# mattsaccount364/FractalShark

Hardware: AMD Instinct MI355X
Metric: Mpix/s (iteration buffer), View #5 3840x2160 HDRx32 LAv2 (higher is better)
Workload: dtype f32+i32exp; 1 GPU; view5_3840x2160_hdrx32_lav2_full; parity=cpu, kernel_variant=tuned, frames=warm: frames of one view back to back

## Files before the change

### fractalshark_amd/csrc/kernels_lav2_hdr32.hip

```cpp
#include <hip/hip_runtime.h>
#include <stdint.h>

#include <type_traits>

#include "../../include/fs_layout.h"
#include "hdr_math.hpp"
#include "at_math.hpp"
#include "kernels.h"
#include <cstdlib>
#include "kernel_common.hpp"
#include "lav2_common.hpp"
#include "scaled_runs.hpp"

using namespace fs;

__global__ void k_test_block_threshold(const int *__restrict__ bw, const int *__restrict__ eshm, const int *__restrict__ sdc,
                                       int *__restrict__ t_out, uint32_t n)
{
    const uint32_t i = blockIdx.x;
    if (i >= n)
        return;
    const int b = __builtin_amdgcn_readfirstlane(bw[i]), e = __builtin_amdgcn_readfirstlane(eshm[i]),
              d = __builtin_amdgcn_readfirstlane(sdc[i]);
    int t;
// ... 19 lines not shown
    if (A.tile_order) {
        const uint32_t w = (blockIdx.y * gridDim.x + blockIdx.x) * (blockDim.x >> 6) + wave_in_block;
        const uint32_t tile = (uint32_t)__builtin_amdgcn_readfirstlane((int)A.tile_order[w]);
        tile_y = tile != 0xFFFFFFFFu ? tile / A.tiles_x : 0u;
        tile_x = tile != 0xFFFFFFFFu ? tile - tile_y * A.tiles_x : 0xFFFFFFFu;
    } else {
        tile_x = blockIdx.x * (blockDim.x >> 6) + wave_in_block;
        tile_y = blockIdx.y;
    }
    uint32_t X, L;
    uint32_t lds_lane16 = 0;
    {
        uint32_t lane;
        asm volatile("v_mbcnt_lo_u32_b32 %0, -1, 0\n\tv_mbcnt_hi_u32_b32 %0, -1, %0" : "=v"(lane));
        X = tile_x * 8u + (lane & 7u);
        L = tile_y * 8u + (lane >> 3);
        if constexpr (kLds)
            asm volatile("v_lshlrev_b32_e32 %0, 4, %1" : "=v"(lds_lane16) : "v"(lane));
    }
    uint32_t lane_cost = 0;
#ifdef FS_TRACE_WAVES
    const uint64_t trace_t0 = wall_clock64();
#endif
    uint64_t c_at = 0, c_la = 0, c_pt = 0, c_px = 0;
    uint64_t c_careful = 0, c_scaled = 0, c_runs = 0;
    uint32_t c_why[4] = {0, 0, 0, 0};
    uint32_t c_nz[4] = {0, 0, 0, 0};
    bool was_skip = false;
    uint32_t c_wentry = 0, c_wstart = 0, c_wshort = 0;
    uint32_t c_blk_violation = 0;
    uint32_t c_pass = 0, c_generic = 0;
    uint32_t c_blk_free = 0, c_blk_tested = 0;
    uint32_t c_lane_steps = 0, c_lane_runs = 0;
#ifdef FS_PROFILE_CYCLES
    uint64_t cyc_loop = 0, cyc_run = 0, cyc_body = 0, cyc_t0 = 0, cyc_t1 = 0, cyc_t2 = 0;
    uint64_t cyc_asm = 0, cyc_tested = 0, cyc_hot = 0, cyc_t3 = 0, cyc_t4 = 0, cyc_t5 = 0, wall_loop = 0, wall_t0 = 0;
#define FS_CYC(stmt) do { if (kStats) { stmt; } } while (0)
#else
#define FS_CYC(stmt) do { } while (0)
#endif
    const uint32_t Y = global_row(A.frame, L);
    const bool live = X < A.frame.width && L < A.frame.local_rows && Y < A.frame.height;
    if (live) {
        c_px = 1;
        const uint32_t n_iterations = A.n_iterations;
        hreal32 deltaReal, deltaImaginary;
        pixel_delta<float>(A.coords, X, Y, deltaReal, deltaImaginary);
        const hcplx32 DeltaSub0 = hc_from_hr(deltaReal, deltaImaginary);
        hcplx32 DeltaSubN = hc_from_native<float>(0.0f, 0.0f);
        uint32_t iterations = 0;
        uint32_t la_cost = 0;

        if (Mode != FS_MODE_PO) {
            if (A.la_valid && A.use_at && hr_cmp_pos(hc_cheb(DeltaSub0), ldr(A.at.ThresholdC)) <= 0) {
                const uint32_t ATMaxIt = n_iterations / A.at.StepLength;
                hcplx32 c = hc_add(hc_mul(DeltaSub0, ldc(A.at.CCoeff)), ldc(A.at.RefC));
                hc_reduce(c);
                hcplx32 z;
                uint32_t i;
                at_perform<float>(c, ldr(A.at.SqrEscapeRadius), ATMaxIt, z, i);
                hcplx32 dz = hc_mul(z, ldc(A.at.InvZCoeff));
                hc_reduce(dz);
                DeltaSubN = dz;
                iterations = i * A.at.StepLength;
                la_cost = i;
                if (kStats)
// ... 86 lines not shown
                pd[0] = dc.re, pd[1] = dc.im, pd[2] = __int_as_float(dc.e);
            }
            int sdc_bits;
            {
                const float mdc = fs_max_abs(dc.re, dc.im);
                const int de = dc.e < -400 ? -400 : (dc.e > 400 ? 400 : dc.e);
                const int lane_bits = mdc > 0.0f ? __float_as_int(__builtin_fmaxf(__builtin_amdgcn_ldexpf(mdc, de), 0x1p-126f))
                                                 : (mdc == 0.0f ? 0 : 0x7f800000);
                sdc_bits = wave_upper_bound_i32(lane_bits);
            }
#define FS_LOAD_DC()                                                                                                \
    f2 dcm;                                                                                                         \
    int dce;                                                                                                        \
    {                                                                                                               \
        uint32_t lane_d;                                                                                            \
        asm volatile("v_mbcnt_lo_u32_b32 %0, -1, 0\n\tv_mbcnt_hi_u32_b32 %0, -1, %0" : "=v"(lane_d));             \
        const uint32_t dc_addr_ = (uint32_t)(uintptr_t)(__attribute__((address_space(3))) float4 *)s_dcp +          \
                                  ((wave_in_block * 64u + lane_d) << 4);                                            \
        typedef float f3l_ __attribute__((ext_vector_type(3)));                                                     \
        f3l_ dc3_;                                                                                                  \
        asm volatile("ds_read_b96 %0, %1\n\ts_waitcnt lgkmcnt(0)" : "=v"(dc3_) : "v"(dc_addr_) : "memory");       \
        dcm = (f2){dc3_.x, dc3_.y};                                                                                 \
        dce = __float_as_int(dc3_.z);                                                                               \
    }
            auto pow2_or_zero = [](int g) -> float {
                return g > -kExpDiffIgnored ? __int_as_float((int)(((uint32_t)g << 23) + 0x3F800000u)) : 0.0f;
            };
            const float4 *__restrict__ zq = A.zq;
            const float4 *__restrict__ zs = A.zs;
            FS_CYC(cyc_t0 = __builtin_readcyclecounter());
            FS_CYC(wall_t0 = wall_clock64());
            uint32_t sc_skip = 0, sc_penalty = 0;
            bool fl_per_trip = false;
            while (running) {
                bool sc_stopped = false;
                if (kScaled && sc_skip != 0u) {
                    bool hot_progress = false, hot_cold = false;
                    FS_CYC(cyc_t5 = __builtin_readcyclecounter());
                    {
                        FS_LOAD_DC()
                        const int E = dze + kScaleShift;
                        const float sE = __builtin_amdgcn_ldexpf(1.0f, E);
                        const f2 sE2 = {sE, sE};
                        const int dsh = dce - E;
                        const f2 dcs = {__builtin_amdgcn_ldexpf(dcm.x, dsh), __builtin_amdgcn_ldexpf(dcm.y, dsh)};
                        const float4 e0 = zs[ref];
                        const float mx0 = fs_max_abs(dzm.x, dzm.y);
                        const float mn0 = fs_min_abs(dzm.x, dzm.y);
                        const bool start_ok = scaled_startable(e0) && mn0 >= FS_FL_FLOOR * __builtin_amdgcn_ldexpf(1.0f, kScaleShift) &&
                                              mx0 >= 1.0f && mx0 < 2.0f && dsh <= 30 - kScaleShift;
                        if (__builtin_amdgcn_ballot_w64(!start_ok) == 0ull) {
                            f2 w = dzm * __builtin_amdgcn_ldexpf(1.0f, -kScaleShift);
                            bool live = true;
#pragma unroll 1
                            for (uint32_t budget = kHotRunSteps; budget != 0u; budget--) {
                                f2 q_, zt;
                                float nz, nq, mxq, mnq, entz;
                                int hb;
                                {
                                    const uint32_t off_ = (live ? ref + 1u : 1u) << 4;
                                    asm volatile("global_load_dwordx2 v[58:59], %[off], %[zs] offset:-16\n\t"
                                                 "global_load_dwordx3 v[60:62], %[off], %[zs]\n\t"
                                                 "s_waitcnt vmcnt(0)\n\t"
                                                 "v_pk_fma_f32 v[56:57], %[w], %[se], v[58:59]\n\t"
                                                 "v_mul_f32_e32 v50, 0.5, v60\n\t"
                                                 "v_pk_mul_f32 v[58:59], %[w], v[56:57] op_sel_hi:[0,1]\n\t"
// ... 119 lines not shown
#define FS_TRIP_FAILED(T, NW_, EB, WSTART)                                                                         \
    {                                                                                                               \
        const float mn_s = fs_min_abs(NW_.x, NW_.y);                         \
        const uint64_t bad_s =                                                                                      \
            __builtin_amdgcn_ballot_w64(__float_as_int(mx_##T) + Esh > __float_as_int(EB)) |                        \
            __builtin_amdgcn_ballot_w64(!(mn_s >= FS_FL_FLOOR));                                                    \
        if (bad_s == 0ull) {                                                                                        \
            wO = NW_;                                                                                               \
            c += 1;                                                                                                 \
        } else {                                                                                                    \
            wO = WSTART;                                                                                            \
        }                                                                                                           \
        failed = true;                                                                                              \
    }
#define FS_TRIP_FAILED_NB(T, NW_, EB, WSTART)                                                                      \
    {                                                                                                               \
        const float mx_s = fs_max_abs(NW_.x, NW_.y);                         \
        const float mn_s = fs_min_abs(NW_.x, NW_.y);                         \
        const uint64_t bad_s =                                                                                      \
            __builtin_amdgcn_ballot_w64(__float_as_int(mx_s) + Esh > __float_as_int(EB)) |                        \
            __builtin_amdgcn_ballot_w64(!(mn_s >= FS_FL_FLOOR));                                                  \
        if (bad_s == 0ull) {                                                                                        \
            wO = NW_;                                                                                               \
            c += 1;                                                                                                 \
        } else {                                                                                                    \
            wO = WSTART;                                                                                            \
        }                                                                                                           \
        failed = true;                                                                                              \
    }
                        f2 w0 = dzm * __builtin_amdgcn_ldexpf(1.0f, -kScaleShift), z0 = {e0.x, e0.y}, w2, z2, wO;
                        uint32_t c = 0;
                        bool failed;
                        FS_CYC(cyc_t2 = __builtin_readcyclecounter());
                        bool fl_redo = false;
                        const uint32_t ref_u = (uint32_t)__builtin_amdgcn_readfirstlane((int)ref);
                        if (__builtin_amdgcn_ballot_w64(ref != ref_u) == 0ull) {
                            if constexpr (kLds) {
                                float4 *wbuf = s_zs_lds + (threadIdx.x >> 6) * 128u;
                                const uint32_t lds_base = (uint32_t)__builtin_amdgcn_readfirstlane(
                                    (int)(uint32_t)(uintptr_t)(__attribute__((address_space(3))) float4 *)wbuf);
                                const uint32_t nchunks = (run_len + 63u) >> 6;
#define FS_GLDS_CHUNK(CH)                                                                                           \
    {                                                                                                               \
        const float4 *src_ = zs + (ref_u + 1u + (CH) * 64u);   \
        const uint32_t dst_ = lds_base + (((CH) & 1u) << 10);                                                       \
        uint32_t keep_;                                                                                             \
        uint64_t exec_;                                                                                             \
        asm volatile("s_or_saveexec_b64 %0, -1\n\t"                                                               \
                     "s_mov_b32 %1, m0\n\t"                                                                       \
                     "s_mov_b32 m0, %3\n\t"                                                                       \
                     "s_nop 0\n\t"                                                                                \
                     "global_load_lds_dwordx4 %2, %4\n\t"                                                         \
                     "s_mov_b32 m0, %1\n\t"                                                                       \
                     "s_mov_b64 exec, %0"                                                                           \
                     : "=&s"(exec_), "=&s"(keep_)                                                                   \
                     : "v"(lds_lane16), "s"(dst_), "s"(src_)                                                        \
                     : "memory", "scc");                                                                            \
    }
                                FS_GLDS_CHUNK(0u)
                                uint32_t chunk = 0;
                                bool run_over = false;
                                while (!run_over) {
                                    if (chunk + 1u < nchunks) {
                                        FS_GLDS_CHUNK(chunk + 1u)
                                        asm volatile("s_waitcnt vmcnt(1)" ::: "memory");
                                    } else {
                                        asm volatile("s_waitcnt vmcnt(0)" ::: "memory");
// ... 31 lines not shown
                                            FS_TRIP_FAILED(e, t5, ue.z, w0)
                                            run_over = true;
                                            break;
                                        }
                                        c += 2;
                                        f2 t7, u7;
                                        uint64_t v4 = 0;
                                        FS_SCALED_STEP(w2, z2, t7, u7, g, v4, false, (void)0, ug.x, ug.y, ug.z);
                                        FS_SCALED_STEP(t7, u7, w0, z0, h, v4, true, (void)0, uh.x, uh.y, uh.z);
                                        if (v4 != 0ull) {
                                            FS_TRIP_FAILED(g, t7, ug.z, w2)
                                            run_over = true;
                                            break;
                                        }
                                        c += 2;
                                    }
                                    if (run_over)
                                        break;
                                    chunk++;
                                    if (c >= run_len) {
                                        wO = w0, failed = false;
                                        run_over = true;
                                    }
                                }
                                asm volatile("s_waitcnt vmcnt(0)" ::: "memory");
#undef FS_GLDS_CHUNK
                            } else {
                            typedef float f4 __attribute__((ext_vector_type(4)));
                            const float4 *zpu = zs + ref_u + 1;
#if defined(FS_VERIFY_BLOCK_BOUND) || defined(FS_VERIFY_FLOOR)
                            const int imdc = __float_as_int(fs_max_abs(dcs.x, dcs.y));
#endif
                            const int Esh_cap = wave_upper_bound_i32(Esh);
                            float mxS = mx0 * __builtin_amdgcn_ldexpf(1.0f, -kScaleShift);
                            int pwi = __builtin_amdgcn_readfirstlane(__float_as_int(e0.w));
                            f2 zS = {__int_as_float(__builtin_amdgcn_readfirstlane(__float_as_int(e0.x))),
                                     __int_as_float(__builtin_amdgcn_readfirstlane(__float_as_int(e0.y)))};
                            f2 wv = w0;
                            uint32_t cs = 0;
                            const uint32_t rl = (uint32_t)__builtin_amdgcn_readfirstlane((int)run_len);
                            const uint32_t lim8 = (rl << 4) - 0x80u;
                            const float4 *const zpb = zpu;
                            for (;;) {
#ifdef FS_VERIFY_BLOCK_BOUND
                                const long long bt_d = (long long)pwi - (long long)Esh_cap;
                                const int bt_thr = sdc_bits > pwi ? -1 : (bt_d > 0x46800000ll ? 0x46800000 : (int)bt_d);
                                const bool bt_pass = __builtin_amdgcn_ballot_w64(__float_as_int(mxS) > bt_thr) == 0ull;
                                if (kStats && bt_pass)
                                    c_blk_free++;
#else
                                {
                                    f2 r1, r2, r3 = wv, ts_, ta_;
                                    uint64_t xacc_ = 0;
                                    float tn_, tl_;
                                    uint64_t msk_;
                                    int st, ebo, pf_, pg_, ph_, bt_t_;
                                    const uint32_t c_in = cs;
                                    uint32_t off = cs << 4;
                                    FS_CYC(cyc_t3 = __builtin_readcyclecounter());
#ifndef FS_VERIFY_FLOOR
                                    if (!fl_per_trip) {
                                        {
                                            FS_FAST_LOOP_FDU(FS_PF_NONE);
                                        }
                                        ebo = 0;
                                    } else
#endif
                                    {
#if !(defined(FS_VERIFY_BLOCK_BOUND) || defined(FS_VERIFY_FLOOR))
                                        const int imdc = __float_as_int(fs_max_abs(dcs.x, dcs.y));
#endif
                                        FS_FAST_LOOP_FL(FS_PF_NONE);
                                    }
#ifdef FS_VERIFY_FLOOR
                                    if (kStats && xacc_ != 0ull)
                                        c_blk_violation++;
#endif
                                    FS_CYC(cyc_asm += __builtin_readcyclecounter() - cyc_t3);
                                    st = __builtin_amdgcn_readfirstlane(st);
                                    zS = (f2){__int_as_float(__builtin_amdgcn_readfirstlane(__float_as_int(zS.x))),
                                              __int_as_float(__builtin_amdgcn_readfirstlane(__float_as_int(zS.y)))};
                                    if (st == 3) {
                                        fl_redo = true;
                                        break;
                                    }
                                    cs = (uint32_t)__builtin_amdgcn_readfirstlane((int)off) >> 4;
                                    pwi = __builtin_amdgcn_readfirstlane(pwi);
                                    if (kStats)
                                        c_blk_free += (cs - c_in) >> 2;
                                    if (st != 0) {
                                        const float ebf = __int_as_float(__builtin_amdgcn_readfirstlane(ebo));
                                        c = cs;
                                        if (st == 1) {
                                            FS_TRIP_FAILED_NB(a, r1, ebf, wv)
                                        } else {
                                            FS_TRIP_FAILED_NB(a, r3, ebf, r2)
                                        }
                                        break;
                                    }
                                }
#endif
                                if (cs + 4u > rl) {
                                    c = cs, wO = wv, failed = false;
                                    break;
                                }
                                if (__builtin_amdgcn_ballot_w64(!(mxS < FS_FL_HIGH)) != 0ull) {
                                    c = cs, wO = wv, failed = false;
                                    break;
                                }
                                if (kStats)
                                    c_blk_tested++;
                                FS_CYC(cyc_t4 = __builtin_readcyclecounter());
                                typedef float f16 __attribute__((ext_vector_type(16)));
                                f16 U;
                                asm volatile("s_load_dwordx16 %0, %1, 0x0" : "=s"(U) : "s"(zpb + cs));
                                f2 tp_, tq_;
                                FS_STEP_ARITH(wv, zS, tp_, a)
                                asm volatile("s_waitcnt lgkmcnt(0)" : "+s"(U), "+v"(tp_));
                                const f4 ua = U.s0123, ub = U.s4567, uc = U.s89ab, ud = U.scdef;
// ... 70 lines not shown
                                FS_SCALED_STEP(w2, z2, t3, u3, c_, v2, false,
                                               asm volatile("s_waitcnt vmcnt(1)" : "+v"(ent_c_), "+v"(mx_c_)), ent_c_.x,
                                               ent_c_.y, ent_c_.z);
                                FS_SCALED_STEP(t3, u3, w0, z0, d, v2, true,
                                               asm volatile("s_waitcnt vmcnt(0)" : "+v"(ent_d), "+v"(mx_d)), ent_d.x,
                                               ent_d.y, ent_d.z);
                                if (v2 != 0ull) {
                                    FS_TRIP_FAILED(c_, t3, ent_c_.z, w2)
                                    break;
                                }
                                c += 2;
                                zp += 4;
                                if (c >= run_len) {
                                    wO = w0, failed = false;
                                    break;
                                }
                            }
                            asm volatile("s_waitcnt vmcnt(0) ; scaled run, loop exit" ::"v"(ent_a), "v"(ent_b), "v"(ent_c_), "v"(ent_d));
                            if (kStats) {
                                c_lane_steps += c;
                                c_lane_runs++;
                            }
                        }
#undef FS_TRIP_FAILED
#undef FS_TRIP_FAILED_NB
                        FS_CYC(cyc_body += __builtin_readcyclecounter() - cyc_t2);
                        if (fl_redo) {
                            uint32_t lane_p;
                            asm volatile("v_mbcnt_lo_u32_b32 %0, -1, 0\n\tv_mbcnt_hi_u32_b32 %0, -1, %0" : "=v"(lane_p));
                            const volatile __attribute__((address_space(3))) float *pz =
                                (const volatile __attribute__((address_space(3))) float *)s_dzp + (wave_in_block * 64u + lane_p) * 2u;
                            dzm = (f2){pz[0], pz[1]};
                            dze = E - kScaleShift;
                            fl_per_trip = true;
                            continue;
                        }
                        fl_per_trip = false;
                        {
                            const float mxw = fs_max_abs(wO.x, wO.y);
                            const int k = (int)((uint32_t)__float_as_int(mxw) >> 23) - 127;
                            dzm = (f2){__builtin_amdgcn_ldexpf(wO.x, -k), __builtin_amdgcn_ldexpf(wO.y, -k)};
                            dze = E + k;
                            ref += c;
                            iterations += c;
                            if (kStats && c != 0u) {
                                c_pt += c;
                                c_scaled += c;
                                c_runs++;
                                c_wstart++;
                                if (c < 8u)
                                    c_wshort++;
                            }
                        }
                        if (failed) {
                            sc_stopped = true;
                            if (c == 0u) {
                                sc_penalty = sc_penalty < kScaledBackoffCap ? sc_penalty + 1u : kScaledBackoffCap;
                                sc_skip = sc_penalty;
                            } else if (c >= 8u) {
                                sc_penalty = 0u;
                            }
                            break;
                        }
                    }
                    FS_CYC(cyc_run += __builtin_readcyclecounter() - cyc_t1);
                }
#define FS_QUIET_STEP(DZM, DZE, ZCM, SC, W, NDZM, NDZE, NZCM, NSC, NW, K, VIOL)                                     \
// ... 236 lines not shown
#ifdef FS_PROFILE_CYCLES
    if (kStats) {
        if ((threadIdx.x & 63) == 0) {
            atomicAdd((unsigned long long *)&A.stats[0], (unsigned long long)cyc_loop);
            atomicAdd((unsigned long long *)&A.stats[1], (unsigned long long)cyc_run);
            atomicAdd((unsigned long long *)&A.stats[3], (unsigned long long)cyc_body);
            atomicAdd((unsigned long long *)&A.stats[24], (unsigned long long)cyc_asm);
            atomicAdd((unsigned long long *)&A.stats[25], (unsigned long long)cyc_tested);
            atomicAdd((unsigned long long *)&A.stats[26], (unsigned long long)cyc_hot);
            atomicAdd((unsigned long long *)&A.stats[27], (unsigned long long)wall_loop);
        }
        c_at = c_la = c_px = 0;
    }
#endif
    if (kStats) {
        add_stats(A.stats, c_at, c_la, c_pt, c_px);
        for (int off = 32; off > 0; off >>= 1) {
            c_careful += __shfl_down(c_careful, off);
            c_scaled += __shfl_down(c_scaled, off);
            c_runs += __shfl_down(c_runs, off);
            const uint32_t bf = __shfl_down(c_blk_free, off), bt = __shfl_down(c_blk_tested, off);
            c_blk_free = bf > c_blk_free ? bf : c_blk_free;
            c_blk_tested = bt > c_blk_tested ? bt : c_blk_tested;
            const uint32_t cp = __shfl_down(c_pass, off), cg = __shfl_down(c_generic, off);
            c_pass = cp > c_pass ? cp : c_pass;
            c_generic = cg > c_generic ? cg : c_generic;
            const uint32_t we = __shfl_down(c_wentry, off), ws = __shfl_down(c_wstart, off), wh = __shfl_down(c_wshort, off);
            c_wentry = we > c_wentry ? we : c_wentry;
            c_wstart = ws > c_wstart ? ws : c_wstart;
            c_wshort = wh > c_wshort ? wh : c_wshort;
            const uint32_t ls = __shfl_down(c_lane_steps, off), lr = __shfl_down(c_lane_runs, off);
            c_lane_steps = ls > c_lane_steps ? ls : c_lane_steps;
            c_lane_runs = lr > c_lane_runs ? lr : c_lane_runs;
            const uint32_t bv = __shfl_down(c_blk_violation, off);
            c_blk_violation = bv > c_blk_violation ? bv : c_blk_violation;
            for (int i = 0; i < 4; i++) {
                const uint32_t y = __shfl_down(c_why[i], off);
                c_why[i] = y > c_why[i] ? y : c_why[i];
                const uint32_t y2 = __shfl_down(c_nz[i], off);
                c_nz[i] = y2 > c_nz[i] ? y2 : c_nz[i];
            }
        }
        if ((threadIdx.x & 63) == 0) {
            atomicAdd((unsigned long long *)&A.stats[5], (unsigned long long)c_careful);
            atomicAdd((unsigned long long *)&A.stats[6], (unsigned long long)c_scaled);
            atomicAdd((unsigned long long *)&A.stats[7], (unsigned long long)c_runs);
            atomicAdd((unsigned long long *)&A.stats[8], (unsigned long long)c_blk_free);
            atomicAdd((unsigned long long *)&A.stats[9], (unsigned long long)c_blk_tested);
            atomicAdd((unsigned long long *)&A.stats[10], (unsigned long long)c_pass);
            atomicAdd((unsigned long long *)&A.stats[11], (unsigned long long)c_generic);
            atomicAdd((unsigned long long *)&A.stats[12], (unsigned long long)c_wentry);
            atomicAdd((unsigned long long *)&A.stats[13], (unsigned long long)c_wstart);
            atomicAdd((unsigned long long *)&A.stats[14], (unsigned long long)c_wshort);
            atomicAdd((unsigned long long *)&A.stats[15], (unsigned long long)c_blk_violation);
            for (int i = 0; i < 4; i++) {
                atomicAdd((unsigned long long *)&A.stats[16 + i], (unsigned long long)c_why[i]);
                atomicAdd((unsigned long long *)&A.stats[20 + i], (unsigned long long)c_nz[i]);
            }
            atomicAdd((unsigned long long *)&A.stats[28], (unsigned long long)c_lane_steps);
            atomicAdd((unsigned long long *)&A.stats[29], (unsigned long long)c_lane_runs);
        }
    }
}
#undef FS_CYC

static dim3 tile_grid(const FsFrame &f) { return dim3((f.width + 31) / 32, (f.local_rows + 7) / 8, 1); }

uint32_t fsk_lav2_hdr32_slots(const FsFrame &f)
{
    return ((f.width + 31u) / 32u) * 4u * ((f.local_rows + 7u) / 8u);
}

void fsk_lav2_hdr32(const FsLav2Args32 &A, int mode, bool stats, int variant, hipStream_t s)
{
    const bool lds_orbit = (variant & FS_VARIANT_FLAG_LDS_ORBIT) != 0;
    variant &= FS_VARIANT_BASE_MASK;
    const dim3 b(256), g = tile_grid(A.frame);
#define FS_LAUNCH_FAST(M, SC, LDS)                                                                                  \
    if (stats) {                                                                                                    \
        if (gs)                                                                                                     \
            hipLaunchKernelGGL((k_lav2_hdr32_fast<M, true, SC, LDS, true>), g, b, 0, s, A);                         \
        else                                                                                                        \
            hipLaunchKernelGGL((k_lav2_hdr32_fast<M, true, SC, LDS, false>), g, b, 0, s, A);                        \
    } else {                                                                                                        \
        if (gs)                                                                                                     \
            hipLaunchKernelGGL((k_lav2_hdr32_fast<M, false, SC, LDS, true>), g, b, 0, s, A);                        \
        else                                                                                                        \
            hipLaunchKernelGGL((k_lav2_hdr32_fast<M, false, SC, LDS, false>), g, b, 0, s, A);                       \
    }
#define FS_LAUNCH(M)                                                                                                \
    do {                                                                                                            \
        if (variant == FS_VARIANT_LITERAL) {                                                                        \
            fsk_lav2_lit32(A, M, stats, g, b, s);                       \
// ... 22 lines not shown
```

### fractalshark_amd/csrc/scaled_runs.hpp

```cpp
#pragma once

#include <hip/hip_runtime.h>
#include <stdint.h>

#include "hdr_math.hpp"
#include "kernels.h"

namespace {

static __device__ __forceinline__ float fs_max_abs(float a, float b)
{
    float r;
    asm("v_max_f32_e64 %0, |%1|, |%2|" : "=v"(r) : "v"(a), "v"(b));
    return r;
}
static __device__ __forceinline__ float fs_min_abs(float a, float b)
{
    float r;
    asm("v_min_f32_e64 %0, |%1|, |%2|" : "=v"(r) : "v"(a), "v"(b));
    return r;
}

}

// ... 133 lines not shown
        "s_branch .Lfl_end_%=\n"                                                                                    \
        ".Lfl_f2_%=:\n\t"                                                                                           \
        "s_mov_b32 %[st], 2\n\t"                                                                                    \
        "s_mov_b32 %[eb], s46\n\t"                                                                                  \
        "s_add_u32 %[off], %[off], 0x20\n\t"                                                                        \
        "s_branch .Lfl_end_%=\n"                                                                                    \
        ".Lfl_f3_%=:\n\t"                                                                                           \
        "s_mov_b32 %[st], 1\n\t"                                                                                    \
        "s_mov_b32 %[eb], s54\n\t"                                                                                  \
        "s_add_u32 %[off], %[off], 0x40\n"                                                                          \
        ".Lfl_end_%=:\n\t"                                                                                          \
        "s_waitcnt lgkmcnt(0)"         \
        : "+{v[48:49]}"(wv), "={v[50:51]}"(r1), "={v[52:53]}"(r2), "+{v[54:55]}"(r3), "={v[56:57]}"(ts_),           \
          "={v[58:59]}"(ta_), "+{v60}"(mxS), "={v61}"(tn_), "={v62}"(tl_), [m] "=&s"(msk_), [st] "=&s"(st),         \
          [eb] "=&s"(ebo), "+{s67}"(pwi), "+{s[64:65]}"(zS), [off] "+s"(off), [pf] "=&s"(pf_), [pg] "=&s"(pg_),     \
          [ph] "=&s"(ph_), [xa] "+s"(xacc_)                                                                         \
        : [se] "v"(sE2), [dc] "v"(dcs), [esh] "v"(Esh), [imdc] "v"(imdc), [lim8] "s"(lim8), "{s[68:69]}"(zpb),      \
          [flr] "s"(kFloorBits), [flr56] "s"((127 - 56) << 23)                                                      \
        : "s36", "s37", "s38", "s39", "s40", "s41", "s42", "s43", "s44", "s45", "s46", "s47", "s48", "s49", "s50",  \
          "s51", "s52", "s53", "s54", "s55", "s56", "s57", "s58", "s59", "s60", "s61", "s62", "s63", "s66", "vcc",  \
          "scc")

#define FS_FL_ACC(A, B) "v_min3_f32 v61, |" A "|, |" B "|, v61\n\t"
#define FS_BT_DC_MAX "v_max_i32_e32 v62, v60, %[imdc]\n\t"
#define FS_BT_DC_ADD "v_add_u32_e32 v62, v62, %[esh]\n\t"

#define FS_BT_T(BW)                                                                                                 \
    "s_sub_i32 %[t], " BW ", %[eshm]\n\t"                                                                           \
    "s_cselect_b32 %[t], 0x46800000, %[t]\n\t"                                                                      \
    "s_min_i32 %[t], %[t], 0x46800000\n\t"                                                                          \
    "s_cmp_gt_i32 %[sdc], " BW "\n\t"                                                                               \
    "s_cselect_b32 %[t], -1, %[t]\n\t"
#define FS_BT_V "v_cmp_lt_i32_e32 vcc, %[t], v60\n\t"
#define FS_FAST_LOOP_FDU(PF)                                                                                        \
    asm volatile(                                                                                                   \
        "v_mov_b32_e32 v61, 0x7f800000\n\t" FS_BT_T("s67") FS_BT_V                                                  \
        ".Lfu_loop_%=:\n\t"          \
        "s_cmp_gt_u32 %[off], %[lim8]\n\t"                                                                          \
        "s_cbranch_scc1 .Lfu_out_%=\n\t"                                                                            \
        "s_cbranch_vccnz .Lfu_out_%=\n\t"                                                         \
        FS_PK_F(FS_R0, "s[64:65]")                                                                                  \
        "s_load_dwordx16 s[36:51], s[68:69], %[off]\n\t"                                                            \
        "s_load_dwordx16 s[52:67], s[68:69], %[off] offset:0x40\n\t"                                                \
        FS_PK_MA(FS_R0) FS_PK_MB(FS_R0) FS_PK_P FS_PK_A(FS_R1)                                                      \
        "s_waitcnt lgkmcnt(0)\n\t" PF FS_BT_T("s51")                                                                \
        FS_PK_F(FS_R1, "s[36:37]") FS_FL_ACC("v50", "v51") FS_PK_MA(FS_R1) FS_PK_MB(FS_R1) FS_PK_P FS_PK_A(FS_R2)   \
        FS_PK_F(FS_R2, "s[40:41]") FS_FL_ACC("v52", "v53") FS_PK_MA(FS_R2) FS_PK_MB(FS_R2) FS_PK_P FS_PK_A(FS_R3)   \
        FS_PK_F(FS_R3, "s[44:45]") FS_FL_ACC("v54", "v55") FS_PK_MA(FS_R3) FS_PK_MB(FS_R3) FS_PK_P FS_PK_A(FS_R0)   \
         \
        FS_PK_F(FS_R0, "s[48:49]") FS_FL_ACC("v48", "v49") FS_PK_MA(FS_R0) FS_T_X("v48", "v49") FS_PK_MB(FS_R0)     \
        FS_PK_P FS_PK_A(FS_R1)                                                                                      \
        FS_PK_F(FS_R1, "s[52:53]") FS_BT_V FS_PK_MA(FS_R1) FS_PK_MB(FS_R1) FS_PK_P                                  \
        "s_cbranch_vccnz .Lfu_blk_%=\n\t" FS_PK_A(FS_R2)                                                            \
        FS_PK_F(FS_R2, "s[56:57]") FS_FL_ACC("v50", "v51") FS_PK_MA(FS_R2) FS_FL_ACC("v52", "v53") FS_PK_MB(FS_R2)  \
        FS_PK_P FS_PK_A(FS_R3)                                                                                      \
        FS_PK_F(FS_R3, "s[60:61]") FS_FL_ACC("v54", "v55") FS_PK_MA(FS_R3) FS_PK_MB(FS_R3) FS_PK_P FS_PK_A(FS_R0)   \
        "s_add_u32 %[off], %[off], 0x80\n\t" FS_BT_T("s67")                                                         \
        FS_T_X("v48", "v49") FS_FL_ACC("v48", "v49") FS_BT_V "s_branch .Lfu_loop_%=\n"                              \
        ".Lfu_blk_%=:\n\t"          \
        "s_mov_b64 s[64:65], s[48:49]\n\t"                                                                          \
        "s_mov_b32 s67, s51\n\t"                                                                                    \
        "s_add_u32 %[off], %[off], 0x40\n"                                                                          \
        ".Lfu_out_%=:\n\t"                                     \
        "s_mov_b32 %[st], 0\n\t" FS_FL_C                                                                            \
        "s_cbranch_vccz .Lfu_end_%=\n\t"                                                                            \
        "s_mov_b32 %[st], 3\n"                                                                                      \
        ".Lfu_end_%=:\n\t"                                                                                          \
        "s_waitcnt lgkmcnt(0)"                                                                                      \
        : "+{v[48:49]}"(wv), "={v[50:51]}"(r1), "={v[52:53]}"(r2), "={v[54:55]}"(r3), "={v[56:57]}"(ts_),           \
          "={v[58:59]}"(ta_), "+{v60}"(mxS), "={v61}"(tn_), [t] "=&s"(bt_t_), [st] "=&s"(st),                       \
          "+{s67}"(pwi), "+{s[64:65]}"(zS), [off] "+s"(off), [pf] "=&s"(pf_), [pg] "=&s"(pg_), [ph] "=&s"(ph_)      \
        : [se] "v"(sE2), [dc] "v"(dcs), [eshm] "s"(Esh_cap), [sdc] "s"(sdc_bits), [lim8] "s"(lim8),                 \
          "{s[68:69]}"(zpb), [flr] "s"(kFloorBits)                                                                  \
        : "s36", "s37", "s38", "s39", "s40", "s41", "s42", "s43", "s44", "s45", "s46", "s47", "s48", "s49", "s50",  \
          "s51", "s52", "s53", "s54", "s55", "s56", "s57", "s58", "s59", "s60", "s61", "s62", "s63", "s66", "vcc",  \
          "scc")

#define FS_FD16_TAIL(EC, ED)                                                                                        \
    FS_PK_F(FS_R2, EC) FS_FL_ACC("v50", "v51") FS_PK_MA(FS_R2) FS_FL_ACC("v52", "v53") FS_PK_MB(FS_R2)              \
    FS_PK_P FS_PK_A(FS_R3)                                                                                          \
    FS_PK_F(FS_R3, ED) FS_FL_ACC("v54", "v55") FS_PK_MA(FS_R3) FS_PK_MB(FS_R3) FS_PK_P FS_PK_A(FS_R0)

#define FS_FD16D_PAIR(EA, EB_, BW, WAIT, LOADS)                                                                     \
    FS_PK_F(FS_R0, EA) FS_FL_ACC("v48", "v49") FS_PK_MA(FS_R0)                                                      \
    "v_max3_f32 v62, |v48|, |v49|, %[imdc]\n\t"                                                                     \
    FS_PK_MB(FS_R0) FS_PK_P                                                                                         \
    "v_subrev_u32_e32 v45, 0x46800000, v62\n\t"                                                                     \
    FS_PK_A(FS_R1)                                                                                                  \
    "v_add_u32_e32 v62, v62, %[esh]\n\t" WAIT                                                                       \
    FS_PK_F(FS_R1, EB_)                                                                                             \
    "v_sub_i32 v62, v62, " BW " clamp\n\t"                                                                          \
    FS_PK_MA(FS_R1)                                                                                                 \
    "v_max3_i32 v63, v63, v62, v45\n\t"                                                                             \
    FS_PK_MB(FS_R1) FS_PK_P LOADS FS_PK_A(FS_R2)
#define FS_FAST_LOOP_FD16P                                                                                          \
    asm volatile(                                                                                                   \
        "v_mov_b32_e32 v61, 0x7f800000\n\t"  \
        "v_bfrev_b32_e32 v63, 1\n\t"                                                                                \
        "s_lshr_b32 %[oc], %[off], 1\n\t"                                                                           \
        "s_load_dwordx16 s[36:51], s[68:69], %[oc]\n\t"                                                             \
        "s_load_dwordx2 s[72:73], s[70:71], %[off]\n"                                                               \
        ".Lfp_loop_%=:\n\t"  \
        "v_sub_u32_e32 v45, %[flr], v61\n\t"                                                                        \
        FS_BT_DC_MAX "s_cmp_gt_u32 %[off], %[lim16]\n\t"                                                            \
        "v_max_i32_e32 v45, v45, v63\n\t"                                                                           \
        FS_BT_DC_ADD                                                                                                \
        "v_cmp_lt_i32_e32 vcc, 0, v45\n\t"                                                                          \
        "s_cbranch_vccnz .Lfp_redo_%=\n\t"                                                 \
        "s_cbranch_scc1 .Lfp_out_%=\n\t"                   \
// ... 140 lines not shown
```

Baseline: 191.2 Mpix/s.

## Add no-dc fast loop variant that drops delta-c add when provably negligible

```diff
diff --git a/fractalshark_amd/csrc/kernels_lav2_hdr32.hip b/fractalshark_amd/csrc/kernels_lav2_hdr32.hip
--- a/fractalshark_amd/csrc/kernels_lav2_hdr32.hip
+++ b/fractalshark_amd/csrc/kernels_lav2_hdr32.hip
@@ -75,6 +75,7 @@
     uint32_t c_pass = 0, c_generic = 0;
     uint32_t c_blk_free = 0, c_blk_tested = 0;
     uint32_t c_lane_steps = 0, c_lane_runs = 0;
+    uint32_t c_nd_steps = 0, c_nd_fail = 0, c_nd_replayed = 0, c_nd_mismatch = 0;
 #ifdef FS_PROFILE_CYCLES
     uint64_t cyc_loop = 0, cyc_run = 0, cyc_body = 0, cyc_t0 = 0, cyc_t1 = 0, cyc_t2 = 0;
     uint64_t cyc_asm = 0, cyc_tested = 0, cyc_hot = 0, cyc_t3 = 0, cyc_t4 = 0, cyc_t5 = 0, wall_loop = 0, wall_t0 = 0;
@@ -227,6 +228,7 @@
             FS_CYC(wall_t0 = wall_clock64());
             uint32_t sc_skip = 0, sc_penalty = 0;
             bool fl_per_trip = false;
+            uint32_t nd_skip = 0;
             while (running) {
                 bool sc_stopped = false;
                 if (kScaled && sc_skip != 0u) {
@@ -412,7 +414,7 @@
                         uint32_t c = 0;
                         bool failed;
                         FS_CYC(cyc_t2 = __builtin_readcyclecounter());
-                        bool fl_redo = false;
+                        bool fl_redo = false, nd_redo = false;
                         const uint32_t ref_u = (uint32_t)__builtin_amdgcn_readfirstlane((int)ref);
                         if (__builtin_amdgcn_ballot_w64(ref != ref_u) == 0ull) {
                             if constexpr (kLds) {
@@ -510,6 +512,19 @@
                             const int imdc = __float_as_int(fs_max_abs(dcs.x, dcs.y));
 #endif
                             const int Esh_cap = wave_upper_bound_i32(Esh);
+                            int nd_form = 0;
+                            if (!fl_per_trip) {
+                                if (nd_skip != 0u) {
+                                    nd_skip--;
+                                } else {
+                                    const float f_run = __builtin_fmaxf(FS_FL_FLOOR, __builtin_amdgcn_ldexpf(fs_max_abs(dcs.x, dcs.y), 26));
+                                    const bool nd_ok = f_run < __builtin_inff() && mn0 * __builtin_amdgcn_ldexpf(1.0f, -kScaleShift) >= f_run;
+                                    if (__builtin_amdgcn_ballot_w64(!nd_ok) == 0ull)
+                                        nd_form = 1;
+                                    else
+                                        nd_skip = kNdBackoffEntry;
+                                }
+                            }
                             float mxS = mx0 * __builtin_amdgcn_ldexpf(1.0f, -kScaleShift);
                             int pwi = __builtin_amdgcn_readfirstlane(__float_as_int(e0.w));
                             f2 zS = {__int_as_float(__builtin_amdgcn_readfirstlane(__float_as_int(e0.x))),
@@ -539,7 +554,42 @@
 #ifndef FS_VERIFY_FLOOR
                                     if (!fl_per_trip) {
                                         {
-                                            FS_FAST_LOOP_FDU(FS_PF_NONE);
+                                            int nd_sel = __builtin_amdgcn_readfirstlane(nd_form);
+                                            if (kStats && nd_form != 0) {
+                                                const f2 wv_s = wv, zS_s = zS;
+                                                const float mxS_s = mxS;
+                                                const int pwi_s = pwi;
+                                                const uint32_t off_s = off;
+                                                FS_FAST_LOOP_FDU(FS_PF_NONE);
+                                                const int st_n = __builtin_amdgcn_readfirstlane(st);
+                                                if (st_n != 5 && st_n != 3) {
+                                                    const f2 wv_n = wv, zS_n = zS;
+                                                    const float mxS_n = mxS;
+                                                    const int pwi_n = pwi;
+                                                    const uint32_t off_n = off;
+                                                    wv = wv_s, zS = zS_s, mxS = mxS_s, pwi = pwi_s, off = off_s;
+                                                    nd_sel = 0;
+                                                    FS_FAST_LOOP_FDU(FS_PF_NONE);
+                                                    const bool lane_diff = __float_as_int(wv.x) != __float_as_int(wv_n.x) ||
+                                                                           __float_as_int(wv.y) != __float_as_int(wv_n.y) ||
+                                                                           __float_as_int(mxS) != __float_as_int(mxS_n);
+                                                    const bool wave_diff =
+                                                        __builtin_amdgcn_readfirstlane(st) != st_n ||
+                                                        __builtin_amdgcn_readfirstlane((int)off) != __builtin_amdgcn_readfirstlane((int)off_n) ||
+                                                        __builtin_amdgcn_readfirstlane(pwi) != __builtin_amdgcn_readfirstlane(pwi_n) ||
+                                                        __builtin_amdgcn_readfirstlane(__float_as_int(zS.x)) !=
+                                                            __builtin_amdgcn_readfirstlane(__float_as_int(zS_n.x)) ||
+                                                        __builtin_amdgcn_readfirstlane(__float_as_int(zS.y)) !=
+                                                            __builtin_amdgcn_readfirstlane(__float_as_int(zS_n.y));
+                                                    c_nd_replayed++;
+                                                    if (wave_diff || __builtin_amdgcn_ballot_w64(lane_diff) != 0ull)
+                                                        c_nd_mismatch++;
+                                                    wv = wv_n, zS = zS_n, mxS = mxS_n, pwi = pwi_n, off = off_n;
+                                                    st = st_n;
+                                                }
+                                            } else {
+                                                FS_FAST_LOOP_FDU(FS_PF_NONE);
+                                            }
                                         }
                                         ebo = 0;
                                     } else
@@ -562,7 +612,15 @@
                                         fl_redo = true;
                                         break;
                                     }
+                                    if (st == 5) {
+                                        fl_redo = nd_redo = true;
+                                        if (kStats)
+                                            c_nd_fail++;
+                                        break;
+                                    }
                                     cs = (uint32_t)__builtin_amdgcn_readfirstlane((int)off) >> 4;
+                                    if (kStats && nd_form != 0)
+                                        c_nd_steps += cs - c_in;
                                     pwi = __builtin_amdgcn_readfirstlane(pwi);
                                     if (kStats)
                                         c_blk_free += (cs - c_in) >> 2;
@@ -699,7 +757,9 @@
                                 (const volatile __attribute__((address_space(3))) float *)s_dzp + (wave_in_block * 64u + lane_p) * 2u;
                             dzm = (f2){pz[0], pz[1]};
                             dze = E - kScaleShift;
-                            fl_per_trip = true;
+                            fl_per_trip = !nd_redo;
+                            if (nd_redo)
+                                nd_skip = kNdBackoffVerdict;
                             continue;
                         }
                         fl_per_trip = false;
@@ -1002,6 +1062,12 @@
             const uint32_t ls = __shfl_down(c_lane_steps, off), lr = __shfl_down(c_lane_runs, off);
             c_lane_steps = ls > c_lane_steps ? ls : c_lane_steps;
             c_lane_runs = lr > c_lane_runs ? lr : c_lane_runs;
+            const uint32_t ns = __shfl_down(c_nd_steps, off), nf = __shfl_down(c_nd_fail, off);
+            c_nd_steps = ns > c_nd_steps ? ns : c_nd_steps;
+            c_nd_fail = nf > c_nd_fail ? nf : c_nd_fail;
+            const uint32_t nr = __shfl_down(c_nd_replayed, off), nm = __shfl_down(c_nd_mismatch, off);
+            c_nd_replayed = nr > c_nd_replayed ? nr : c_nd_replayed;
+            c_nd_mismatch = nm > c_nd_mismatch ? nm : c_nd_mismatch;
             const uint32_t bv = __shfl_down(c_blk_violation, off);
             c_blk_violation = bv > c_blk_violation ? bv : c_blk_violation;
             for (int i = 0; i < 4; i++) {
@@ -1029,6 +1095,10 @@
             }
             atomicAdd((unsigned long long *)&A.stats[28], (unsigned long long)c_lane_steps);
             atomicAdd((unsigned long long *)&A.stats[29], (unsigned long long)c_lane_runs);
+            atomicAdd((unsigned long long *)&A.stats[30], (unsigned long long)c_nd_steps);
+            atomicAdd((unsigned long long *)&A.stats[32], (unsigned long long)c_nd_fail);
+            atomicAdd((unsigned long long *)&A.stats[33], (unsigned long long)c_nd_mismatch);
+            atomicAdd((unsigned long long *)&A.stats[34], (unsigned long long)c_nd_replayed);
         }
     }
 }
diff --git a/fractalshark_amd/csrc/scaled_runs.hpp b/fractalshark_amd/csrc/scaled_runs.hpp
--- a/fractalshark_amd/csrc/scaled_runs.hpp
+++ b/fractalshark_amd/csrc/scaled_runs.hpp
@@ -189,49 +189,67 @@
     "s_cmp_gt_i32 %[sdc], " BW "\n\t"                                                                               \
     "s_cselect_b32 %[t], -1, %[t]\n\t"
 #define FS_BT_V "v_cmp_lt_i32_e32 vcc, %[t], v60\n\t"
+#define FS_PK_PN(NW) "v_pk_add_f32 " NW ", v[58:59], v[56:57] neg_lo:[0,1] neg_hi:[0,0]\n\t"
+#define FS_FDU_LOOP(L, PF, PRE, POST)                                                                               \
+        ".L" L "_loop_%=:\n\t"       \
+        "s_cmp_gt_u32 %[off], %[lim8]\n\t"                                                                          \
+        "s_cbranch_scc1 .L" L "_out_%=\n\t"                                                                         \
+        "s_cbranch_vccnz .L" L "_out_%=\n\t"                                                      \
+        FS_PK_F(FS_R0, "s[64:65]")                                                                                  \
+        "s_load_dwordx16 s[36:51], s[68:69], %[off]\n\t"                                                            \
+        "s_load_dwordx16 s[52:67], s[68:69], %[off] offset:0x40\n\t"                                                \
+        FS_PK_MA(FS_R0) FS_PK_MB(FS_R0) PRE POST(FS_R1)                                                             \
+        "s_waitcnt lgkmcnt(0)\n\t" PF FS_BT_T("s51")                                                                \
+        FS_PK_F(FS_R1, "s[36:37]") FS_FL_ACC("v50", "v51") FS_PK_MA(FS_R1) FS_PK_MB(FS_R1) PRE POST(FS_R2)          \
+        FS_PK_F(FS_R2, "s[40:41]") FS_FL_ACC("v52", "v53") FS_PK_MA(FS_R2) FS_PK_MB(FS_R2) PRE POST(FS_R3)          \
+        FS_PK_F(FS_R3, "s[44:45]") FS_FL_ACC("v54", "v55") FS_PK_MA(FS_R3) FS_PK_MB(FS_R3) PRE POST(FS_R0)          \
+         \
+        FS_PK_F(FS_R0, "s[48:49]") FS_FL_ACC("v48", "v49") FS_PK_MA(FS_R0) FS_T_X("v48", "v49") FS_PK_MB(FS_R0)     \
+        PRE POST(FS_R1)                                                                                             \
+        FS_PK_F(FS_R1, "s[52:53]") FS_BT_V FS_PK_MA(FS_R1) FS_PK_MB(FS_R1) PRE                                      \
+        "s_cbranch_vccnz .L" L "_blk_%=\n\t" POST(FS_R2)                                                            \
+        FS_PK_F(FS_R2, "s[56:57]") FS_FL_ACC("v50", "v51") FS_PK_MA(FS_R2) FS_FL_ACC("v52", "v53") FS_PK_MB(FS_R2)  \
+        PRE POST(FS_R3)                                                                                             \
+        FS_PK_F(FS_R3, "s[60:61]") FS_FL_ACC("v54", "v55") FS_PK_MA(FS_R3) FS_PK_MB(FS_R3) PRE POST(FS_R0)          \
+        "s_add_u32 %[off], %[off], 0x80\n\t" FS_BT_T("s67")                                                         \
+        FS_T_X("v48", "v49") FS_FL_ACC("v48", "v49") FS_BT_V "s_branch .L" L "_loop_%=\n"                           \
+        ".L" L "_blk_%=:\n\t"        \
+        "s_mov_b64 s[64:65], s[48:49]\n\t"                                                                          \
+        "s_mov_b32 s67, s51\n\t"                                                                                    \
+        "s_add_u32 %[off], %[off], 0x40\n"                                                                          \
+        ".L" L "_out_%=:\n\t"
 #define FS_FAST_LOOP_FDU(PF)                                                                                        \
     asm volatile(                                                                                                   \
         "v_mov_b32_e32 v61, 0x7f800000\n\t" FS_BT_T("s67") FS_BT_V                                                  \
-        ".Lfu_loop_%=:\n\t"          \
-        "s_cmp_gt_u32 %[off], %[lim8]\n\t"                                                                          \
-        "s_cbranch_scc1 .Lfu_out_%=\n\t"                                                                            \
-        "s_cbranch_vccnz .Lfu_out_%=\n\t"                                                         \
-        FS_PK_F(FS_R0, "s[64:65]")                                                                                  \
-        "s_load_dwordx16 s[36:51], s[68:69], %[off]\n\t"                                                            \
-        "s_load_dwordx16 s[52:67], s[68:69], %[off] offset:0x40\n\t"                                                \
-        FS_PK_MA(FS_R0) FS_PK_MB(FS_R0) FS_PK_P FS_PK_A(FS_R1)                                                      \
-        "s_waitcnt lgkmcnt(0)\n\t" PF FS_BT_T("s51")                                                                \
-        FS_PK_F(FS_R1, "s[36:37]") FS_FL_ACC("v50", "v51") FS_PK_MA(FS_R1) FS_PK_MB(FS_R1) FS_PK_P FS_PK_A(FS_R2)   \
-        FS_PK_F(FS_R2, "s[40:41]") FS_FL_ACC("v52", "v53") FS_PK_MA(FS_R2) FS_PK_MB(FS_R2) FS_PK_P FS_PK_A(FS_R3)   \
-        FS_PK_F(FS_R3, "s[44:45]") FS_FL_ACC("v54", "v55") FS_PK_MA(FS_R3) FS_PK_MB(FS_R3) FS_PK_P FS_PK_A(FS_R0)   \
-         \
-        FS_PK_F(FS_R0, "s[48:49]") FS_FL_ACC("v48", "v49") FS_PK_MA(FS_R0) FS_T_X("v48", "v49") FS_PK_MB(FS_R0)     \
-        FS_PK_P FS_PK_A(FS_R1)                                                                                      \
-        FS_PK_F(FS_R1, "s[52:53]") FS_BT_V FS_PK_MA(FS_R1) FS_PK_MB(FS_R1) FS_PK_P                                  \
-        "s_cbranch_vccnz .Lfu_blk_%=\n\t" FS_PK_A(FS_R2)                                                            \
-        FS_PK_F(FS_R2, "s[56:57]") FS_FL_ACC("v50", "v51") FS_PK_MA(FS_R2) FS_FL_ACC("v52", "v53") FS_PK_MB(FS_R2)  \
-        FS_PK_P FS_PK_A(FS_R3)                                                                                      \
-        FS_PK_F(FS_R3, "s[60:61]") FS_FL_ACC("v54", "v55") FS_PK_MA(FS_R3) FS_PK_MB(FS_R3) FS_PK_P FS_PK_A(FS_R0)   \
-        "s_add_u32 %[off], %[off], 0x80\n\t" FS_BT_T("s67")                                                         \
-        FS_T_X("v48", "v49") FS_FL_ACC("v48", "v49") FS_BT_V "s_branch .Lfu_loop_%=\n"                              \
-        ".Lfu_blk_%=:\n\t"          \
-        "s_mov_b64 s[64:65], s[48:49]\n\t"                                                                          \
-        "s_mov_b32 s67, s51\n\t"                                                                                    \
-        "s_add_u32 %[off], %[off], 0x40\n"                                                                          \
-        ".Lfu_out_%=:\n\t"                                     \
+        "s_cmp_lg_u32 %[nd], 0\n\t"                                                                                 \
+        "s_cbranch_scc1 .Lfn_loop_%=\n"                                                                             \
+        FS_FDU_LOOP("fu", PF, FS_PK_P, FS_PK_A)                \
         "s_mov_b32 %[st], 0\n\t" FS_FL_C                                                                            \
         "s_cbranch_vccz .Lfu_end_%=\n\t"                                                                            \
+        "s_mov_b32 %[st], 3\n\t"                                                                                    \
+        "s_branch .Lfu_end_%=\n"                                                                                    \
+        FS_FDU_LOOP("fn", PF, "", FS_PK_PN)             \
+        "v_max_f32_e64 v62, |%[dcx]|, |%[dcy]|\n\t"                                                                 \
+        "s_mov_b32 %[st], 0\n\t"                                                                                    \
+        "v_ldexp_f32 v62, v62, 26\n\t"                                                                              \
+        "v_max_f32_e32 v62, %[flr], v62\n\t"                                                                        \
+        "v_cmp_gt_f32_e32 vcc, v62, v61\n\t"                                                                        \
+        "s_cbranch_vccz .Lfu_end_%=\n\t"  \
+        "s_mov_b32 %[st], 5\n\t" FS_FL_C                                                                            \
+        "s_cbranch_vccz .Lfu_end_%=\n\t"                                                                            \
         "s_mov_b32 %[st], 3\n"                                                                                      \
-        ".Lfu_end_%=:\n\t"                                                                                          \
+        ".Lfu_end_%=:\n\t"                                                                                        \
         "s_waitcnt lgkmcnt(0)"                                                                                      \
         : "+{v[48:49]}"(wv), "={v[50:51]}"(r1), "={v[52:53]}"(r2), "={v[54:55]}"(r3), "={v[56:57]}"(ts_),           \
-          "={v[58:59]}"(ta_), "+{v60}"(mxS), "={v61}"(tn_), [t] "=&s"(bt_t_), [st] "=&s"(st),                       \
+          "={v[58:59]}"(ta_), "+{v60}"(mxS), "={v61}"(tn_), "={v62}"(tl_), [t] "=&s"(bt_t_), [st] "=&s"(st),        \
           "+{s67}"(pwi), "+{s[64:65]}"(zS), [off] "+s"(off), [pf] "=&s"(pf_), [pg] "=&s"(pg_), [ph] "=&s"(ph_)      \
-        : [se] "v"(sE2), [dc] "v"(dcs), [eshm] "s"(Esh_cap), [sdc] "s"(sdc_bits), [lim8] "s"(lim8),                 \
-          "{s[68:69]}"(zpb), [flr] "s"(kFloorBits)                                                                  \
+        : [se] "v"(sE2), [dc] "v"(dcs), [dcx] "v"(dcs.x), [dcy] "v"(dcs.y), [eshm] "s"(Esh_cap),                    \
+          [sdc] "s"(sdc_bits), [lim8] "s"(lim8), [nd] "s"(nd_sel), "{s[68:69]}"(zpb), [flr] "s"(kFloorBits)         \
         : "s36", "s37", "s38", "s39", "s40", "s41", "s42", "s43", "s44", "s45", "s46", "s47", "s48", "s49", "s50",  \
           "s51", "s52", "s53", "s54", "s55", "s56", "s57", "s58", "s59", "s60", "s61", "s62", "s63", "s66", "vcc",  \
           "scc")
+constexpr uint32_t kNdBackoffEntry = 8;
+constexpr uint32_t kNdBackoffVerdict = 32;
 
 #define FS_FD16_TAIL(EC, ED)                                                                                        \
     FS_PK_F(FS_R2, EC) FS_FL_ACC("v50", "v51") FS_PK_MA(FS_R2) FS_FL_ACC("v52", "v53") FS_PK_MB(FS_R2)              \
```

Result: faster. 209.9 Mpix/s, median of 6 (+9.8%).
